# neonbjb/tortoise-tts

Hardware: NVIDIA H100
Metric: audio-seconds/sec at preset='standard' (higher is better)
Workload: dtype bf16 tensor-core operands, fp32 accumulate/residual/norm/softmax/scheduler

## Files before the change

### tortoise_tts_b200/csrc/common.cuh

```cuda
#pragma once
#include <cuda_runtime.h>
#include <cuda_bf16.h>
#include <cuda.h>
#include <stdint.h>
#include <cstdlib>

#define TTB_DEVINL __device__ __forceinline__

namespace ttb {

void set_error(const char* fmt, ...);
int check_cuda(cudaError_t e, const char* what);
#define TTB_CHECK_LAUNCH(what)                                   \
  do {                                                           \
    cudaError_t _e = cudaGetLastError();                         \
    if (_e != cudaSuccess) return ttb::check_cuda(_e, what);     \
  } while (0)

TTB_DEVINL void pdl_wait() { asm volatile("griddepcontrol.wait;" ::: "memory"); }
TTB_DEVINL void pdl_launch_dependents() { asm volatile("griddepcontrol.launch_dependents;" ::: "memory"); }

inline bool pdl_enabled() {
  static int v = -1;
  if (v < 0) {
// ... 46 lines not shown
  __syncthreads();
  if (lane == 0) red[w] = v;
  __syncthreads();
  float r = (lane < nw) ? red[lane] : 0.f;
  r = warp_sum(r);
  return r;
}
TTB_DEVINL float block_max(float v, float* red) {
  int lane = threadIdx.x & 31, w = threadIdx.x >> 5, nw = (blockDim.x + 31) >> 5;
  v = warp_max(v);
  __syncthreads();
  if (lane == 0) red[w] = v;
  __syncthreads();
  float r = (lane < nw) ? red[lane] : -INFINITY;
  r = warp_max(r);
  return r;
}

TTB_DEVINL uint32_t pack_bf16(float a, float b) {
  __nv_bfloat162 t = __floats2bfloat162_rn(a, b);
  return *reinterpret_cast<uint32_t*>(&t);
}
TTB_DEVINL float2 unpack_bf16(uint32_t u) {
  __nv_bfloat162 t = *reinterpret_cast<__nv_bfloat162*>(&u);
  return __bfloat1622float2(t);
}

TTB_DEVINL uint32_t smem_u32(const void* p) { return static_cast<uint32_t>(__cvta_generic_to_shared(p)); }

TTB_DEVINL unsigned long long global_timer_ns() {
  unsigned long long t;
  asm volatile("mov.u64 %0, %%globaltimer;" : "=l"(t));
  return t;
}
TTB_DEVINL unsigned long long sm_id() {
  uint32_t s;
  asm volatile("mov.u32 %0, %%smid;" : "=r"(s));
  return s;
}

TTB_DEVINL bool elect_one() {
  uint32_t pred = 0;
  asm volatile(
      "{\n\t.reg .pred P;\n\t.reg .b32 R;\n\t"
      "elect.sync R|P, 0xffffffff;\n\t"
      "selp.u32 %0, 1, 0, P;\n\t}\n"
      : "=r"(pred));
  return pred != 0;
}

TTB_DEVINL void mbar_init(uint64_t* bar, uint32_t count) {
  asm volatile("mbarrier.init.shared::cta.b64 [%0], %1;" ::"r"(smem_u32(bar)), "r"(count));
}
TTB_DEVINL void fence_barrier_init() { asm volatile("fence.mbarrier_init.release.cluster;" ::: "memory"); }
TTB_DEVINL void fence_proxy_async() { asm volatile("fence.proxy.async.shared::cta;" ::: "memory"); }
TTB_DEVINL void mbar_arrive_expect_tx(uint64_t* bar, uint32_t bytes) {
  asm volatile("mbarrier.arrive.expect_tx.shared::cta.b64 _, [%0], %1;" ::"r"(smem_u32(bar)), "r"(bytes) : "memory");
}
TTB_DEVINL void mbar_arrive(uint64_t* bar) {
  asm volatile("mbarrier.arrive.shared::cta.b64 _, [%0];" ::"r"(smem_u32(bar)) : "memory");
}
#ifndef TTB_MBAR_HINT_NS
#define TTB_MBAR_HINT_NS 20000
#endif
TTB_DEVINL void mbar_wait(uint64_t* bar, uint32_t parity) {
#if TTB_MBAR_HINT_NS > 0
  asm volatile(
      "{\n\t.reg .pred P1;\n\t"
      "WAIT_LOOP:\n\t"
      "mbarrier.try_wait.parity.shared::cta.b64 P1, [%0], %1, %2;\n\t"
      "@P1 bra DONE;\n\t"
      "bra WAIT_LOOP;\n\t"
      "DONE:\n\t}\n" ::"r"(smem_u32(bar)),
      "r"(parity), "r"((uint32_t)TTB_MBAR_HINT_NS)
      : "memory");
#else
  asm volatile(
      "{\n\t.reg .pred P1;\n\t"
      "WAIT_LOOP:\n\t"
      "mbarrier.try_wait.parity.shared::cta.b64 P1, [%0], %1;\n\t"
      "@P1 bra DONE;\n\t"
      "bra WAIT_LOOP;\n\t"
      "DONE:\n\t}\n" ::"r"(smem_u32(bar)),
      "r"(parity)
      : "memory");
#endif
}

TTB_DEVINL void tma_prefetch_desc(const CUtensorMap* m) {
  asm volatile("prefetch.tensormap [%0];" ::"l"(reinterpret_cast<uint64_t>(m)) : "memory");
}
TTB_DEVINL void tma_load_2d(void* smem_dst, const CUtensorMap* map, uint64_t* bar, int c0, int c1) {
  asm volatile(
      "cp.async.bulk.tensor.2d.shared::cluster.global.mbarrier::complete_tx::bytes [%0], [%1, {%3, %4}], [%2];"
      ::"r"(smem_u32(smem_dst)), "l"(reinterpret_cast<uint64_t>(map)), "r"(smem_u32(bar)), "r"(c0), "r"(c1)
      : "memory");
}
TTB_DEVINL void tma_load_3d(void* smem_dst, const CUtensorMap* map, uint64_t* bar, int c0, int c1, int c2) {
  asm volatile(
      "cp.async.bulk.tensor.3d.shared::cluster.global.mbarrier::complete_tx::bytes [%0], [%1, {%3, %4, %5}], [%2];"
      ::"r"(smem_u32(smem_dst)), "l"(reinterpret_cast<uint64_t>(map)), "r"(smem_u32(bar)), "r"(c0), "r"(c1), "r"(c2)
      : "memory");
}
TTB_DEVINL void tma_prefetch_l2_3d(const CUtensorMap* map, int c0, int c1, int c2) {
  asm volatile("cp.async.bulk.prefetch.tensor.3d.L2.global.tile [%0, {%1, %2, %3}];"
               ::"l"(reinterpret_cast<uint64_t>(map)), "r"(c0), "r"(c1), "r"(c2)
               : "memory");
}

TTB_DEVINL void wgmma_fence() { asm volatile("wgmma.fence.sync.aligned;" ::: "memory"); }
TTB_DEVINL void wgmma_commit() { asm volatile("wgmma.commit_group.sync.aligned;" ::: "memory"); }
template <int N>
TTB_DEVINL void wgmma_wait() { asm volatile("wgmma.wait_group.sync.aligned %0;" ::"n"(N) : "memory"); }
TTB_DEVINL void named_barrier(int id, int nthreads) { asm volatile("bar.sync %0, %1;" ::"r"(id), "r"(nthreads) : "memory"); }

TTB_DEVINL uint64_t wgmma_desc_kmajor_sw128(uint32_t smem_addr) {
  uint64_t d = 0;
  d |= (uint64_t)((smem_addr & 0x3FFFF) >> 4);
  d |= (uint64_t)1 << 16;
  d |= (uint64_t)(1024 >> 4) << 32;
  d |= (uint64_t)1 << 62;
  return d;
}
TTB_DEVINL uint64_t wgmma_desc_mnmajor_sw128(uint32_t smem_addr, uint32_t lbo_bytes) {
  uint64_t d = 0;
  d |= (uint64_t)((smem_addr & 0x3FFFF) >> 4);
  d |= (uint64_t)((lbo_bytes >> 4) & 0x3FFF) << 16;
  d |= (uint64_t)(1024 >> 4) << 32;
  d |= (uint64_t)1 << 62;
  return d;
}

TTB_DEVINL void wgmma_m64n16k16_bf16_ss(float* d, uint64_t desc_a, uint64_t desc_b, uint32_t scale_d) {
  asm volatile(
      "{\n\t.reg .pred p;\n\tsetp.ne.b32 p, %10, 0;\n\t"
      "wgmma.mma_async.sync.aligned.m64n16k16.f32.bf16.bf16 {%0, %1, %2, %3, %4, %5, %6, %7}, %8, %9, p, 1, 1, 0, 0;\n\t}\n"
      : "+f"(d[0]), "+f"(d[1]), "+f"(d[2]), "+f"(d[3]), "+f"(d[4]), "+f"(d[5]), "+f"(d[6]), "+f"(d[7])
      : "l"(desc_a), "l"(desc_b), "r"(scale_d));
}
TTB_DEVINL void wgmma_m64n32k16_bf16_ss(float* d, uint64_t desc_a, uint64_t desc_b, uint32_t scale_d) {
  asm volatile(
      "{\n\t.reg .pred p;\n\tsetp.ne.b32 p, %18, 0;\n\t"
      "wgmma.mma_async.sync.aligned.m64n32k16.f32.bf16.bf16 {%0, %1, %2, %3, %4, %5, %6, %7, %8, %9, %10, %11, %12, %13, %14, %15}, %16, %17, p, 1, 1, 0, 0;\n\t}\n"
      : "+f"(d[0]), "+f"(d[1]), "+f"(d[2]), "+f"(d[3]), "+f"(d[4]), "+f"(d[5]), "+f"(d[6]), "+f"(d[7]), "+f"(d[8]), "+f"(d[9]), "+f"(d[10]), "+f"(d[11]), "+f"(d[12]), "+f"(d[13]), "+f"(d[14]), "+f"(d[15])
      : "l"(desc_a), "l"(desc_b), "r"(scale_d));
}
TTB_DEVINL void wgmma_m64n64k16_bf16_ss(float* d, uint64_t desc_a, uint64_t desc_b, uint32_t scale_d) {
  asm volatile(
      "{\n\t.reg .pred p;\n\tsetp.ne.b32 p, %34, 0;\n\t"
      "wgmma.mma_async.sync.aligned.m64n64k16.f32.bf16.bf16 {%0, %1, %2, %3, %4, %5, %6, %7, %8, %9, %10, %11, %12, %13, %14, %15, %16, %17, %18, %19, %20, %21, %22, %23, %24, %25, %26, %27, %28, %29, %30, %31}, %32, %33, p, 1, 1, 0, 0;\n\t}\n"
      : "+f"(d[0]), "+f"(d[1]), "+f"(d[2]), "+f"(d[3]), "+f"(d[4]), "+f"(d[5]), "+f"(d[6]), "+f"(d[7]), "+f"(d[8]), "+f"(d[9]), "+f"(d[10]), "+f"(d[11]), "+f"(d[12]), "+f"(d[13]), "+f"(d[14]), "+f"(d[15]), "+f"(d[16]), "+f"(d[17]), "+f"(d[18]), "+f"(d[19]), "+f"(d[20]), "+f"(d[21]), "+f"(d[22]), "+f"(d[23]), "+f"(d[24]), "+f"(d[25]), "+f"(d[26]), "+f"(d[27]), "+f"(d[28]), "+f"(d[29]), "+f"(d[30]), "+f"(d[31])
      : "l"(desc_a), "l"(desc_b), "r"(scale_d));
}
template <int TNSPB>
TTB_DEVINL void wgmma_m64n64k16_bf16_rs(float* d, const uint32_t* a, uint64_t desc_b, uint32_t scale_d) {
  asm volatile(
      "{\n\t.reg .pred p;\n\tsetp.ne.b32 p, %37, 0;\n\t"
      "wgmma.mma_async.sync.aligned.m64n64k16.f32.bf16.bf16 {%0, %1, %2, %3, %4, %5, %6, %7, %8, %9, %10, %11, %12, %13, %14, %15, %16, %17, %18, %19, %20, %21, %22, %23, %24, %25, %26, %27, %28, %29, %30, %31}, {%32, %33, %34, %35}, %36, p, 1, 1, %38;\n\t}\n"
      : "+f"(d[0]), "+f"(d[1]), "+f"(d[2]), "+f"(d[3]), "+f"(d[4]), "+f"(d[5]), "+f"(d[6]), "+f"(d[7]), "+f"(d[8]), "+f"(d[9]), "+f"(d[10]), "+f"(d[11]), "+f"(d[12]), "+f"(d[13]), "+f"(d[14]), "+f"(d[15]), "+f"(d[16]), "+f"(d[17]), "+f"(d[18]), "+f"(d[19]), "+f"(d[20]), "+f"(d[21]), "+f"(d[22]), "+f"(d[23]), "+f"(d[24]), "+f"(d[25]), "+f"(d[26]), "+f"(d[27]), "+f"(d[28]), "+f"(d[29]), "+f"(d[30]), "+f"(d[31])
      : "r"(a[0]), "r"(a[1]), "r"(a[2]), "r"(a[3]), "l"(desc_b), "r"(scale_d), "n"(TNSPB));
}

template <int BN>
TTB_DEVINL void gemm_mma_kblock(float* acc, uint32_t sa, uint32_t sb, bool first) {
  wgmma_fence();
#pragma unroll
  for (int k = 0; k < 4; ++k) {
    const uint64_t da = wgmma_desc_kmajor_sw128(sa + k * 32);
    const uint32_t sc = (first && k == 0) ? 0u : 1u;
    if constexpr (BN == 32) {
      wgmma_m64n32k16_bf16_ss(acc, da, wgmma_desc_kmajor_sw128(sb + k * 32), sc);
    } else {
#pragma unroll
      for (int nb = 0; nb < BN / 64; ++nb)
        wgmma_m64n64k16_bf16_ss(acc + nb * 32, da, wgmma_desc_kmajor_sw128(sb + nb * 8192 + k * 32), sc);
    }
  }
  wgmma_commit();
}

}
```

### tortoise_tts_b200/csrc/gemm.cu

```cuda
#include "common.cuh"
#include "ttb_internal.h"

#include <map>
#include <mutex>
#include <string>
#include <vector>
#include <cstring>

namespace ttb {

typedef CUresult (*PFN_encodeTiled)(CUtensorMap*, CUtensorMapDataType, cuuint32_t, void*, const cuuint64_t*,
                                    const cuuint64_t*, const cuuint32_t*, const cuuint32_t*, CUtensorMapInterleave,
                                    CUtensorMapSwizzle, CUtensorMapL2promotion, CUtensorMapFloatOOBfill);

static PFN_encodeTiled get_encode_fn() {
  static PFN_encodeTiled fn = nullptr;
  static std::once_flag once;
  std::call_once(once, []() {
    void* p = nullptr;
    cudaDriverEntryPointQueryResult q;
    if (cudaGetDriverEntryPoint("cuTensorMapEncodeTiled", &p, cudaEnableDefault, &q) == cudaSuccess &&
        q == cudaDriverEntryPointSuccess)
      fn = reinterpret_cast<PFN_encodeTiled>(p);
  });
// ... 158 lines not shown
          tma_load_3d(sb, &map_b, &full_bar[kbi], tap * K + kk, n0, 0);
        } else if (ep.wpre > 1) {
          tma_prefetch_l2_3d(&map_b, tap * K + kk, n0, 0);
        } else {
          break;
        }
      }
    }
  }
  pdl_wait();
  if (tr && threadIdx.x == 0) tr[2] = global_timer_ns();

  if (warp == PRODUCER_WARP) {
    if (lane == 0 || (SPLIT_PRODUCER && lane == 1)) {
      int stage = 0; uint32_t phase = 0;
      for (int kbi = 0; kbi < pre; ++kbi) {
        const int kb = kb_begin + kbi;
        const int tap = kb / kblocks_per_tap;
        const int kk = (kb - tap * kblocks_per_tap) * BK;
        tma_load_3d(smem + kbi * L::STAGE_BYTES, &map_a, &full_bar[kbi], kk, m0 + tap * ep.tap_dil - pad, bz * a_batch_mul);
        if (++stage == STAGES) { stage = 0; phase ^= 1; }
      }
      for (int kbi = pre; kbi < num_kb; ++kbi) {
        mbar_wait(&empty_bar[stage], phase ^ 1);
        const int kb = kb_begin + kbi;
        const int tap = kb / kblocks_per_tap;
        const int kk = (kb - tap * kblocks_per_tap) * BK;
        uint8_t* sa = smem + stage * L::STAGE_BYTES;
        uint8_t* sb = sa + L::A_BYTES;
        if constexpr (SPLIT_PRODUCER) {
          if (lane == 0) {
            mbar_arrive_expect_tx(&full_bar[stage], L::A_BYTES);
            tma_load_3d(sa, &map_a, &full_bar[stage], kk, m0 + tap * ep.tap_dil - pad, bz * a_batch_mul);
          } else {
            mbar_arrive_expect_tx(&full_bar[stage], L::B_BYTES);
            tma_load_3d(sb, &map_b, &full_bar[stage], tap * K + kk, n0, 0);
          }
        } else {
          mbar_arrive_expect_tx(&full_bar[stage], L::STAGE_BYTES);
          tma_load_3d(sa, &map_a, &full_bar[stage], kk, m0 + tap * ep.tap_dil - pad, bz * a_batch_mul);
          tma_load_3d(sb, &map_b, &full_bar[stage], tap * K + kk, n0, 0);
        }
        if (++stage == STAGES) { stage = 0; phase ^= 1; }
      }
    }
    __syncwarp();
    pdl_launch_dependents();
  } else {
    const int wg = warp >> 2;
    const int rb = warp >> 1;
    if (ep.residual) {
      const int m = m0 + rb * 32 + lane;
      if (m < M && !(warp & 1)) {
        const float* p = ep.residual + (long long)bz * ep.res_bstride + (long long)m * ep.ldr + n0;
#pragma unroll
        for (int c = 0; c < BN; c += 32)
          if (n0 + c < N) asm volatile("prefetch.global.L2 [%0];" ::"l"(p + c));
      }
    }
    float acc[BN / 2];
    int stage = 0; uint32_t phase = 0;
    if (tr && threadIdx.x == 0) tr[3] = global_timer_ns();
    gemm_consumer_mainloop<BN, STAGES>(acc, smem, L::STAGE_BYTES, L::A_BYTES, full_bar, empty_bar, num_kb, stage, phase, wg,
                                       (threadIdx.x & 127) == 0, [](uint64_t* b) { mbar_arrive(b); });
    if (tr && threadIdx.x == 0) tr[4] = global_timer_ns();
    pdl_launch_dependents();
    named_barrier(1, GEMM_CONSUMERS);
    gemm_stage_accumulator<BN>(acc, smem_u32(smem), warp, lane);
    named_barrier(1, GEMM_CONSUMERS);
    if (tr && threadIdx.x == 0) tr[5] = global_timer_ns();
    gemm_epilogue_dispatch<BN>(smem_u32(smem) + (uint32_t)(rb * 32 * (BN + 8)) * 4, n0, N, m0 + rb * 32, M, lane, (long long)bz,
                               ep, warp & 1, 2);
    if (tr && threadIdx.x == 0) tr[6] = global_timer_ns();
  }
  __syncthreads();
  if (tr && threadIdx.x == 0) tr[7] = global_timer_ns();
}

__global__ void gemm_ref_kernel(const __nv_bfloat16* A, long long a_bstride, int lda, int rows, const __nv_bfloat16* W,
                                int M, int N, int K, int taps, int pad, GemmEpilogue ep) {
  const int n = blockIdx.x * blockDim.x + threadIdx.x;
  const int m = blockIdx.y;
  const int bz = blockIdx.z;
  if (n >= N || m >= M) return;
  const int nn = (ep.act == TTB_ACT_GEGLU) ? (n & ~1) : n;
  float acc[2] = {0.f, 0.f};
  const int cnt = (ep.act == TTB_ACT_GEGLU) ? 2 : 1;
  if (ep.act == TTB_ACT_GEGLU && (n & 1)) return;
  for (int c = 0; c < cnt; ++c) {
    float s = 0.f;
    for (int tap = 0; tap < taps; ++tap) {
      const int r = m + tap - pad;
      if (r < 0 || r >= rows) continue;
      const __nv_bfloat16* a = A + (long long)bz * a_bstride + (long long)r * lda;
      const __nv_bfloat16* w = W + (long long)(nn + c) * taps * K + (long long)tap * K;
      for (int k = 0; k < K; ++k) s += __bfloat162float(a[k]) * __bfloat162float(w[k]);
    }
    s *= ep.alpha;
    if (ep.bias) s += ep.bias[nn + c];
    acc[c] = s;
  }
  float v;
  int on = n;
  if (ep.act == TTB_ACT_GEGLU) { v = acc[0] * gelu_erf(acc[1]); on = n >> 1; }
  else {
    v = acc[0];
    if (ep.act == TTB_ACT_GELU_NEW) v = gelu_new(v);
    else if (ep.act == TTB_ACT_SILU) v = silu(v);
    else if (ep.act == TTB_ACT_LRELU02) v = leaky(v, 0.2f);
    else if (ep.act == TTB_ACT_GELU_ERF) v = gelu_erf(v);
    if (ep.residual) v += ep.residual[(long long)bz * ep.res_bstride + (long long)m * ep.ldr + n];
  }
  if (ep.out_f32) ep.out_f32[(long long)bz * ep.outf_bstride + (long long)m * ep.ldo + on] = v;
  if (ep.out_bf16) ep.out_bf16[(long long)bz * ep.outb_bstride + (long long)m * ep.ldob + on] = __float2bfloat16(v);
}

static int g_gemm_impl = -1;
static unsigned long long* g_gemm_trace = nullptr;

template <int BN, int STAGES, bool SPLIT_PRODUCER = false>
static int launch_tc(const TtbGemmArgs& g, const GemmEpilogue& ep, cudaStream_t st) {
  CUtensorMap ma, mb;
  const bool bcast = (g.batch == 1) || (g.a_bstride == 0);
  const uint64_t a_d2 = bcast ? 1 : (uint64_t)g.batch;
  const uint64_t a_s2 = bcast ? (uint64_t)g.rows * g.lda : (uint64_t)g.a_bstride;
  if (get_tensor_map_bf16(&ma, g.A, (uint64_t)g.K, (uint64_t)g.rows, a_d2, (uint64_t)g.lda, a_s2, BK, BM)) return -1;
  if (get_tensor_map_bf16(&mb, g.W, (uint64_t)g.K * g.taps, (uint64_t)g.N, 1, (uint64_t)g.K * g.taps,
                          (uint64_t)g.K * g.taps * g.N, BK, BN)) return -1;
  using L = GemmSmem<BN, STAGES>;
  static bool attr_set = false;
  if (!attr_set) {
    cudaError_t e = cudaFuncSetAttribute(gemm_bf16_tc_kernel<BN, STAGES, SPLIT_PRODUCER>, cudaFuncAttributeMaxDynamicSharedMemorySize, L::TOTAL);
    if (e != cudaSuccess) return check_cuda(e, "cudaFuncSetAttribute(gemm)");
    attr_set = true;
  }
  int kb_per_split = 0, zdim = g.batch;
  if (g.splitk > 1) {
    const int kb_total = (g.K / BK) * g.taps;
    kb_per_split = (kb_total + g.splitk - 1) / g.splitk;
    zdim = (kb_total + kb_per_split - 1) / kb_per_split;
  }
  dim3 grid((g.N + BN - 1) / BN, (g.M + BM - 1) / BM, zdim);
  cudaError_t le = launch_pdl(gemm_bf16_tc_kernel<BN, STAGES, SPLIT_PRODUCER>, grid, dim3(GEMM_THREADS), (size_t)L::TOTAL, st, ma, mb, g.M, g.N,
                              g.K, g.taps, g.pad, (bcast || g.splitk > 1) ? 0 : 1, kb_per_split, ep, g_gemm_trace);
  if (le != cudaSuccess) return check_cuda(le, "gemm_bf16_tc_kernel launch");
  TTB_CHECK_LAUNCH("gemm_bf16_tc_kernel");
  return 0;
}

}

#include "gemm_persist.cuh"
#include "gemm_mc.cuh"

namespace ttb {

static int num_sms() {
  static int n = 0;
  if (!n) {
    int dev = 0;
    cudaGetDevice(&dev);
    cudaDeviceGetAttribute(&n, cudaDevAttrMultiProcessorCount, dev);
    if (n <= 0) n = 132;
  }
  return n;
}

template <int BN, int PSTAGES>
static int launch_persistent(const TtbGemmArgs& g, const GemmEpilogue& ep, cudaStream_t st) {
  CUtensorMap ma, mb;
  const bool bcast = (g.batch == 1) || (g.a_bstride == 0);
  const uint64_t a_d2 = bcast ? 1 : (uint64_t)g.batch;
  const uint64_t a_s2 = bcast ? (uint64_t)g.rows * g.lda : (uint64_t)g.a_bstride;
  if (get_tensor_map_bf16(&ma, g.A, (uint64_t)g.K, (uint64_t)g.rows, a_d2, (uint64_t)g.lda, a_s2, BK, BM)) return -1;
  if (get_tensor_map_bf16(&mb, g.W, (uint64_t)g.K * g.taps, (uint64_t)g.N, 1, (uint64_t)g.K * g.taps,
                          (uint64_t)g.K * g.taps * g.N, BK, BN)) return -1;
  using L = GemmPSmem<BN, PSTAGES>;
  static bool attr_set = false;
  if (!attr_set) {
    cudaError_t e = cudaFuncSetAttribute(gemm_bf16_tc_persistent_kernel<BN, PSTAGES>,
                                         cudaFuncAttributeMaxDynamicSharedMemorySize, L::TOTAL);
    if (e != cudaSuccess) return check_cuda(e, "cudaFuncSetAttribute(gemm persistent)");
    attr_set = true;
  }
  int kb_per_split = 0, zdim = g.batch;
  if (g.splitk > 1) {
    const int kb_total = (g.K / BK) * g.taps;
    kb_per_split = (kb_total + g.splitk - 1) / g.splitk;
    zdim = (kb_total + kb_per_split - 1) / kb_per_split;
  }
  const int m_tiles = (g.M + BM - 1) / BM, n_tiles = (g.N + BN - 1) / BN;
  const long long total = (long long)m_tiles * n_tiles * zdim;
  const int grid = (int)(total < num_sms() ? total : num_sms());
  const cudaError_t le = launch_pdl(gemm_bf16_tc_persistent_kernel<BN, PSTAGES>, dim3(grid), dim3(GEMM_THREADS), (size_t)L::TOTAL, st,
      ma, mb, g.M, g.N, g.K, g.taps, g.pad, (bcast || g.splitk > 1) ? 0 : 1, kb_per_split, m_tiles, n_tiles, zdim, ep);
  if (le != cudaSuccess) return check_cuda(le, "gemm_bf16_tc_persistent_kernel launch");
  TTB_CHECK_LAUNCH("gemm_bf16_tc_persistent_kernel");
  return 0;
}

}

using namespace ttb;

extern "C" int ttb_debug_gemm_trace(void* buf) {
  g_gemm_trace = static_cast<unsigned long long*>(buf);
  return 0;
}

extern "C" int ttb_gemm(const TtbGemmArgs* gp, void* stream) {
  const TtbGemmArgs& g = *gp;
  cudaStream_t st = static_cast<cudaStream_t>(stream);
  if (g.K % BK != 0 || g.K <= 0) { set_error("ttb_gemm: K=%d must be a positive multiple of 64", g.K); return -1; }
  if (g.taps < 1 || g.M <= 0 || g.N <= 0 || g.batch <= 0) { set_error("ttb_gemm: bad shape"); return -1; }
  if (g.act == TTB_ACT_GEGLU && (g.N & 1)) { set_error("ttb_gemm: GEGLU needs even N"); return -1; }
  GemmEpilogue ep;
  ep.bias = g.bias; ep.residual = g.residual; ep.out_f32 = g.out_f32;
  ep.out_bf16 = reinterpret_cast<__nv_bfloat16*>(g.out_bf16);
  ep.res_bstride = g.res_bstride; ep.outf_bstride = g.outf_bstride; ep.outb_bstride = g.outb_bstride;
  ep.ldr = g.ldr; ep.ldo = g.ldo; ep.ldob = g.ldob; ep.act = g.act; ep.alpha = g.alpha;
  ep.gn_part = nullptr; ep.gn_groups = g.gn_groups;
  static int wpre_on = -1;
  if (wpre_on < 0) { const char* e = getenv("TTB_GEMM_WPREFETCH"); wpre_on = e ? atoi(e) : 1; }
  ep.wpre = g.w_static ? wpre_on : 0;
  ep.tap_dil = g.tap_dilation > 1 ? g.tap_dilation : 1;
  if (ep.tap_dil > 1 && (g.cluster > 1 || g.variant == 6 || g.force_ref || g_gemm_impl == 1)) {
    set_error("ttb_gemm: tap_dilation is implemented by the one-tile and the persistent kernels only");
    return -1;
  }
  if (g.gn_partials) {
    if (g.N != 32 * g.gn_groups || (g.M + 31) / 32 > TTB_GN_SPLITS || g.act == TTB_ACT_GEGLU || g.splitk > 1 || g.force_ref) {
      set_error("ttb_gemm: gn_partials needs N == 32 * gn_groups, M <= %d, no GEGLU / split-K (N=%d groups=%d M=%d)",
                32 * TTB_GN_SPLITS, g.N, g.gn_groups, g.M);
      return -1;
    }
    ep.gn_part = reinterpret_cast<float2*>(g.gn_partials + 16);
  }
  if (g_gemm_impl < 0) {
    const char* e = getenv("TTB_GEMM_IMPL");
    g_gemm_impl = (e && strcmp(e, "ref") == 0) ? 1 : 0;
  }
  if (g.splitk > 1) {
    if (g.batch != 1 || g.act != TTB_ACT_NONE || !g.out_f32 || g.out_bf16 || g.bias || g.residual) {
      set_error("ttb_gemm: splitk needs batch=1, no activation/bias/residual and an fp32 partial buffer");
      return -1;
    }
    if (g_gemm_impl == 1 || g.force_ref) { set_error("ttb_gemm: splitk is not available in the SIMT checker"); return -1; }
  }
  if (g_gemm_impl == 1 || g.force_ref) {
    dim3 block(128), grid((g.N + 127) / 128, g.M, g.batch);
    gemm_ref_kernel<<<grid, block, 0, st>>>(reinterpret_cast<const __nv_bfloat16*>(g.A), g.a_bstride, g.lda, g.rows,
                                            reinterpret_cast<const __nv_bfloat16*>(g.W), g.M, g.N, g.K, g.taps, g.pad, ep);
    TTB_CHECK_LAUNCH("gemm_ref_kernel");
    return 0;
  }
  const long long tiles128 = (long long)((g.N + 127) / 128) * ((g.M + BM - 1) / BM) * g.batch;
  if (g.cluster > 1) {
    const int bn = g.tile_n == 32 ? 32 : (g.tile_n == 64 ? 64 : 128);
    const int n_tiles = (g.N + bn - 1) / bn;
    if ((g.cluster != 2 && g.cluster != 4) || n_tiles % g.cluster != 0) {
      set_error("ttb_gemm: cluster=%d needs 2 or 4 and a multiple of it in N tiles (%d)", g.cluster, n_tiles);
      return -1;
    }
    if (bn == 32) return g.cluster == 4 ? launch_mc<32, 4, 4>(g, ep, st) : launch_mc<32, 4, 2>(g, ep, st);
    if (bn == 64) return g.cluster == 4 ? launch_mc<64, 4, 4>(g, ep, st) : launch_mc<64, 4, 2>(g, ep, st);
    return g.cluster == 4 ? launch_mc<128, 3, 4>(g, ep, st) : launch_mc<128, 3, 2>(g, ep, st);
  }
  if (g.variant == 6) { set_error("ttb_gemm: variant 6 (CTA-pair MMA) needs hardware this library does not target"); return -1; }
  static int persist = -1;
  if (persist < 0) { const char* e = getenv("TTB_GEMM_PERSIST"); persist = e ? atoi(e) : 0; }
  if (g.variant == 2) {
    if (g.tile_n == 32) return launch_persistent<32, 8>(g, ep, st);
    if (g.tile_n == 64) return launch_persistent<64, 6>(g, ep, st);
    return launch_persistent<128, 4>(g, ep, st);
  }
  const int use_persist = (g.variant == 1) ? 0 : persist;
  if (use_persist && g.tile_n == 0 && tiles128 >= 2 * num_sms()) return launch_persistent<128, 4>(g, ep, st);
  if (use_persist == 2) {
    if (g.tile_n == 32) return launch_persistent<32, 8>(g, ep, st);
    if (g.tile_n == 64 || (g.tile_n == 0 && tiles128 < num_sms())) return launch_persistent<64, 6>(g, ep, st);
    if (g.tile_n != 256) return launch_persistent<128, 4>(g, ep, st);
  }
  if (g.tile_n == 32) {
    static int t32 = -1;
    if (t32 < 0) { const char* e = getenv("TTB_GEMM_T32_STAGES"); t32 = e ? atoi(e) : 5; }
    return (g.variant == 3 || (g.variant != 4 && t32 == 5)) ? launch_tc<32, 5>(g, ep, st) : launch_tc<32, 4>(g, ep, st);
  }
  if (g.tile_n == 64 && g.variant == 3) return launch_tc<64, 8>(g, ep, st);
  if (g.tile_n == 64 || (g.tile_n == 0 && tiles128 < num_sms())) return launch_tc<64, 4>(g, ep, st);
  if (g.tile_n == 256) return launch_tc<256, 3>(g, ep, st);
  if (g.variant == 5) return launch_tc<128, 3, true>(g, ep, st);
  return launch_tc<128, 3>(g, ep, st);
}
```

### tortoise_tts_b200/csrc/gemm_epilogue.cuh

```cuda
#pragma once

namespace ttb {

TTB_DEVINL float4 lds128(uint32_t addr) {
  float4 v;
  asm volatile("ld.shared.v4.f32 {%0, %1, %2, %3}, [%4];" : "=f"(v.x), "=f"(v.y), "=f"(v.z), "=f"(v.w) : "r"(addr) : "memory");
  return v;
}

template <int BN>
TTB_DEVINL void gemm_stage_accumulator(const float* acc, uint32_t tile, int cwarp, int lane) {
  constexpr int PITCH = BN + 8;
  const uint32_t base = tile + (uint32_t)((cwarp * 16 + (lane >> 2)) * PITCH + 2 * (lane & 3)) * 4;
#pragma unroll
  for (int i = 0; i < BN / 2; i += 4) {
    asm volatile("st.shared.v2.f32 [%0], {%1, %2};" ::"r"(base + (uint32_t)(2 * i) * 4), "f"(acc[i]), "f"(acc[i + 1]) : "memory");
    asm volatile("st.shared.v2.f32 [%0], {%1, %2};" ::"r"(base + (uint32_t)(8 * PITCH + 2 * i) * 4), "f"(acc[i + 2]), "f"(acc[i + 3]) : "memory");
  }
}

template <int ACT>
TTB_DEVINL float epi_act(float x) {
  if (ACT == TTB_ACT_GELU_NEW) return gelu_new(x);
  if (ACT == TTB_ACT_SILU) return silu(x);
  if (ACT == TTB_ACT_LRELU02) return leaky(x, 0.2f);
  if (ACT == TTB_ACT_TANH) return tanhf(x);
  if (ACT == TTB_ACT_GELU_ERF) return gelu_erf(x);
  return x;
}

struct EpiFlags {
  bool aligned;
};

TTB_DEVINL EpiFlags epi_flags(const GemmEpilogue& ep) {
  EpiFlags f;
  f.aligned = (!ep.bias || (reinterpret_cast<uintptr_t>(ep.bias) & 15) == 0) &&
              (!ep.residual || ((ep.ldr & 3) == 0 && (ep.res_bstride & 3) == 0 && (reinterpret_cast<uintptr_t>(ep.residual) & 15) == 0)) &&
              (!ep.out_f32 || ((ep.ldo & 3) == 0 && (ep.outf_bstride & 3) == 0 && (reinterpret_cast<uintptr_t>(ep.out_f32) & 15) == 0)) &&
              (!ep.out_bf16 || ((ep.ldob & 3) == 0 && (ep.outb_bstride & 3) == 0 && (reinterpret_cast<uintptr_t>(ep.out_bf16) & 7) == 0));
  return f;
}

TTB_DEVINL void epi_gn_store(float gs, float gq, int nb, int m_base, int lane, long long bz, const GemmEpilogue& ep) {
#pragma unroll
  for (int off = 16; off > 0; off >>= 1) {
    gs += __shfl_xor_sync(0xffffffffu, gs, off);
    gq += __shfl_xor_sync(0xffffffffu, gq, off);
  }
  if (lane == 0)
    ep.gn_part[((long long)bz * ep.gn_groups + (nb >> 5)) * TTB_GN_SPLITS + (m_base >> 5)] = make_float2(gs, gq);
}

template <int ACT>
TTB_DEVINL void epi_chunk_fast(uint32_t blk, int pitch, int nb, int m_base, int rows_valid, int lane, long long bz,
                               const GemmEpilogue& ep) {
  const bool GN = ep.gn_part != nullptr;
  const int rr0 = lane >> 3, c = (lane & 7) * 4;
  float4 b = make_float4(0.f, 0.f, 0.f, 0.f);
  if (ep.bias) b = __ldg(reinterpret_cast<const float4*>(ep.bias + nb + c));
  if (ACT == TTB_ACT_GEGLU) {
    const long long col = (nb >> 1) + (c >> 1);
#pragma unroll
    for (int it = 0; it < 8; ++it) {
      const int rr = it * 4 + rr0;
      const float4 a = lds128(blk + (uint32_t)(rr * pitch + c) * 4);
      const float o0 = fmaf(a.x, ep.alpha, b.x) * gelu_erf(fmaf(a.y, ep.alpha, b.y));
      const float o1 = fmaf(a.z, ep.alpha, b.z) * gelu_erf(fmaf(a.w, ep.alpha, b.w));
      const long long m = m_base + rr;
      if (rr >= rows_valid) continue;
      if (ep.out_bf16) *reinterpret_cast<uint32_t*>(ep.out_bf16 + bz * ep.outb_bstride + m * ep.ldob + col) = pack_bf16(o0, o1);
      if (ep.out_f32) *reinterpret_cast<float2*>(ep.out_f32 + bz * ep.outf_bstride + m * ep.ldo + col) = make_float2(o0, o1);
    }
    return;
  }
  const long long col = nb + c;
  float4 rs[8];
  if (ep.residual) {
    const float* rp = ep.residual + bz * ep.res_bstride + (long long)(m_base + rr0) * ep.ldr + col;
#pragma unroll
    for (int it = 0; it < 8; ++it) {
      if (it * 4 + rr0 < rows_valid) rs[it] = *reinterpret_cast<const float4*>(rp + (long long)it * 4 * ep.ldr);
      else rs[it] = make_float4(0.f, 0.f, 0.f, 0.f);
    }
  }
  float gs = 0.f, gq = 0.f;
#pragma unroll
  for (int it = 0; it < 8; ++it) {
    const int rr = it * 4 + rr0;
    const float4 a = lds128(blk + (uint32_t)(rr * pitch + c) * 4);
    float4 o;
    o.x = epi_act<ACT>(fmaf(a.x, ep.alpha, b.x));
    o.y = epi_act<ACT>(fmaf(a.y, ep.alpha, b.y));
    o.z = epi_act<ACT>(fmaf(a.z, ep.alpha, b.z));
    o.w = epi_act<ACT>(fmaf(a.w, ep.alpha, b.w));
    if (ep.residual) { o.x += rs[it].x; o.y += rs[it].y; o.z += rs[it].z; o.w += rs[it].w; }
    const long long m = m_base + rr;
    if (rr >= rows_valid) continue;
    if (ep.out_f32) *reinterpret_cast<float4*>(ep.out_f32 + bz * ep.outf_bstride + m * ep.ldo + col) = o;
    if (ep.out_bf16)
      *reinterpret_cast<uint2*>(ep.out_bf16 + bz * ep.outb_bstride + m * ep.ldob + col) = make_uint2(pack_bf16(o.x, o.y), pack_bf16(o.z, o.w));
    if (GN) {
      gs += (o.x + o.y) + (o.z + o.w);
      gq += (o.x * o.x + o.y * o.y) + (o.z * o.z + o.w * o.w);
    }
  }
  if (GN) epi_gn_store(gs, gq, nb, m_base, lane, bz, ep);
}

template <int ACT>
TTB_DEVINL void epi_chunk_slow(const uint32_t* r, int nb, int N, int m, int M, long long bz, const GemmEpilogue& ep,
                               float& gs, float& gq) {
  if (m >= M) return;
  if (ACT == TTB_ACT_GEGLU) {
    const int nout = N >> 1, ob = nb >> 1;
    float* of = ep.out_f32 ? ep.out_f32 + bz * ep.outf_bstride + (long long)m * ep.ldo : nullptr;
    __nv_bfloat16* obf = ep.out_bf16 ? ep.out_bf16 + bz * ep.outb_bstride + (long long)m * ep.ldob : nullptr;
#pragma unroll
    for (int j = 0; j < 16; ++j) {
      if (ob + j < nout) {
        float u = __uint_as_float(r[2 * j]) * ep.alpha, g = __uint_as_float(r[2 * j + 1]) * ep.alpha;
        if (ep.bias) { u += __ldg(ep.bias + nb + 2 * j); g += __ldg(ep.bias + nb + 2 * j + 1); }
        const float o = u * gelu_erf(g);
        if (of) of[ob + j] = o;
        if (obf) obf[ob + j] = __float2bfloat16(o);
      }
    }
    return;
  }
  const float* rp = ep.residual ? ep.residual + bz * ep.res_bstride + (long long)m * ep.ldr : nullptr;
  float* of = ep.out_f32 ? ep.out_f32 + bz * ep.outf_bstride + (long long)m * ep.ldo : nullptr;
  __nv_bfloat16* obf = ep.out_bf16 ? ep.out_bf16 + bz * ep.outb_bstride + (long long)m * ep.ldob : nullptr;
#pragma unroll
  for (int j = 0; j < 32; ++j) {
    if (nb + j < N) {
      float x = __uint_as_float(r[j]) * ep.alpha;
      if (ep.bias) x += __ldg(ep.bias + nb + j);
      x = epi_act<ACT>(x);
      if (rp) x += rp[nb + j];
      if (of) of[nb + j] = x;
      if (obf) obf[nb + j] = __float2bfloat16(x);
      gs += x;
      gq += x * x;
    }
  }
}

template <int BN, int ACT>
TTB_DEVINL void gemm_epilogue_tile(uint32_t blk, int n0, int N, int m_base, int M, int lane, long long bz,
                                   const GemmEpilogue& ep, int ch_begin, int ch_step) {
  constexpr int NCH = BN / 32;
  constexpr int PITCH = BN + 8;
  const bool aligned = epi_flags(ep).aligned;
  const int rows_valid = min(32, M - m_base);
#pragma unroll 1
  for (int ch = ch_begin; ch < NCH; ch += ch_step) {
    const int nb = n0 + ch * 32;
    if (nb >= N || rows_valid <= 0) continue;
    if (aligned && nb + 32 <= N) {
      epi_chunk_fast<ACT>(blk + (uint32_t)ch * 128, PITCH, nb, m_base, rows_valid, lane, bz, ep);
    } else {
      uint32_t r[32];
#pragma unroll
      for (int j = 0; j < 8; ++j) {
        const float4 a = lds128(blk + (uint32_t)(lane * PITCH + ch * 32 + 4 * j) * 4);
        r[4 * j] = __float_as_uint(a.x); r[4 * j + 1] = __float_as_uint(a.y);
        r[4 * j + 2] = __float_as_uint(a.z); r[4 * j + 3] = __float_as_uint(a.w);
      }
      float gs = 0.f, gq = 0.f;
      epi_chunk_slow<ACT>(r, nb, N, m_base + lane, M, bz, ep, gs, gq);
      if (ep.gn_part) epi_gn_store(gs, gq, nb, m_base, lane, bz, ep);
    }
  }
}

template <int BN>
TTB_DEVINL void gemm_epilogue_dispatch(uint32_t blk, int n0, int N, int m_base, int M, int lane, long long bz,
                                       const GemmEpilogue& ep, int ch_begin, int ch_step) {
  switch (ep.act) {
    case TTB_ACT_GEGLU: gemm_epilogue_tile<BN, TTB_ACT_GEGLU>(blk, n0, N, m_base, M, lane, bz, ep, ch_begin, ch_step); break;
    case TTB_ACT_GELU_NEW: gemm_epilogue_tile<BN, TTB_ACT_GELU_NEW>(blk, n0, N, m_base, M, lane, bz, ep, ch_begin, ch_step); break;
    case TTB_ACT_SILU: gemm_epilogue_tile<BN, TTB_ACT_SILU>(blk, n0, N, m_base, M, lane, bz, ep, ch_begin, ch_step); break;
    case TTB_ACT_LRELU02: gemm_epilogue_tile<BN, TTB_ACT_LRELU02>(blk, n0, N, m_base, M, lane, bz, ep, ch_begin, ch_step); break;
    case TTB_ACT_TANH: gemm_epilogue_tile<BN, TTB_ACT_TANH>(blk, n0, N, m_base, M, lane, bz, ep, ch_begin, ch_step); break;
    case TTB_ACT_GELU_ERF: gemm_epilogue_tile<BN, TTB_ACT_GELU_ERF>(blk, n0, N, m_base, M, lane, bz, ep, ch_begin, ch_step); break;
    default: gemm_epilogue_tile<BN, TTB_ACT_NONE>(blk, n0, N, m_base, M, lane, bz, ep, ch_begin, ch_step); break;
  }
}

}
```

Measured before the change: 6.990.

## Add warp-specialised persistent 128x256 WGMMA GEMM with register reallocation

Adds a persistent, warp-specialised GEMM kernel. One producer warpgroup issues TMA loads, while two consumer warpgroups each run m64n256k16 WGMMA across a 4-stage mbarrier pipeline. setmaxnreg moves registers from the producer to the consumers. The epilogue is staged through shared memory in 32-column slices. The kernel is on by default for non-split-K GEMMs whose 128x128 tile count fills the SMs; it aims to improve tensor-core utilisation and overlap loads with MMA. The cost is heavy register pressure from 128 accumulator floats per thread, and an epilogue that does not overlap with the next tile's mainloop.

After: 7.380 (median of 6 runs). 1.06x the previous value.

```diff
diff --git a/tortoise_tts_b200/csrc/common.cuh b/tortoise_tts_b200/csrc/common.cuh
--- a/tortoise_tts_b200/csrc/common.cuh
+++ b/tortoise_tts_b200/csrc/common.cuh
@@ -222,6 +222,13 @@
       : "+f"(d[0]), "+f"(d[1]), "+f"(d[2]), "+f"(d[3]), "+f"(d[4]), "+f"(d[5]), "+f"(d[6]), "+f"(d[7]), "+f"(d[8]), "+f"(d[9]), "+f"(d[10]), "+f"(d[11]), "+f"(d[12]), "+f"(d[13]), "+f"(d[14]), "+f"(d[15]), "+f"(d[16]), "+f"(d[17]), "+f"(d[18]), "+f"(d[19]), "+f"(d[20]), "+f"(d[21]), "+f"(d[22]), "+f"(d[23]), "+f"(d[24]), "+f"(d[25]), "+f"(d[26]), "+f"(d[27]), "+f"(d[28]), "+f"(d[29]), "+f"(d[30]), "+f"(d[31])
       : "l"(desc_a), "l"(desc_b), "r"(scale_d));
 }
+TTB_DEVINL void wgmma_m64n256k16_bf16_ss(float* d, uint64_t desc_a, uint64_t desc_b, uint32_t scale_d) {
+  asm volatile(
+      "{\n\t.reg .pred p;\n\tsetp.ne.b32 p, %130, 0;\n\t"
+      "wgmma.mma_async.sync.aligned.m64n256k16.f32.bf16.bf16 {%0, %1, %2, %3, %4, %5, %6, %7, %8, %9, %10, %11, %12, %13, %14, %15, %16, %17, %18, %19, %20, %21, %22, %23, %24, %25, %26, %27, %28, %29, %30, %31, %32, %33, %34, %35, %36, %37, %38, %39, %40, %41, %42, %43, %44, %45, %46, %47, %48, %49, %50, %51, %52, %53, %54, %55, %56, %57, %58, %59, %60, %61, %62, %63, %64, %65, %66, %67, %68, %69, %70, %71, %72, %73, %74, %75, %76, %77, %78, %79, %80, %81, %82, %83, %84, %85, %86, %87, %88, %89, %90, %91, %92, %93, %94, %95, %96, %97, %98, %99, %100, %101, %102, %103, %104, %105, %106, %107, %108, %109, %110, %111, %112, %113, %114, %115, %116, %117, %118, %119, %120, %121, %122, %123, %124, %125, %126, %127}, %128, %129, p, 1, 1, 0, 0;\n\t}\n"
+      : "+f"(d[0]), "+f"(d[1]), "+f"(d[2]), "+f"(d[3]), "+f"(d[4]), "+f"(d[5]), "+f"(d[6]), "+f"(d[7]), "+f"(d[8]), "+f"(d[9]), "+f"(d[10]), "+f"(d[11]), "+f"(d[12]), "+f"(d[13]), "+f"(d[14]), "+f"(d[15]), "+f"(d[16]), "+f"(d[17]), "+f"(d[18]), "+f"(d[19]), "+f"(d[20]), "+f"(d[21]), "+f"(d[22]), "+f"(d[23]), "+f"(d[24]), "+f"(d[25]), "+f"(d[26]), "+f"(d[27]), "+f"(d[28]), "+f"(d[29]), "+f"(d[30]), "+f"(d[31]), "+f"(d[32]), "+f"(d[33]), "+f"(d[34]), "+f"(d[35]), "+f"(d[36]), "+f"(d[37]), "+f"(d[38]), "+f"(d[39]), "+f"(d[40]), "+f"(d[41]), "+f"(d[42]), "+f"(d[43]), "+f"(d[44]), "+f"(d[45]), "+f"(d[46]), "+f"(d[47]), "+f"(d[48]), "+f"(d[49]), "+f"(d[50]), "+f"(d[51]), "+f"(d[52]), "+f"(d[53]), "+f"(d[54]), "+f"(d[55]), "+f"(d[56]), "+f"(d[57]), "+f"(d[58]), "+f"(d[59]), "+f"(d[60]), "+f"(d[61]), "+f"(d[62]), "+f"(d[63]), "+f"(d[64]), "+f"(d[65]), "+f"(d[66]), "+f"(d[67]), "+f"(d[68]), "+f"(d[69]), "+f"(d[70]), "+f"(d[71]), "+f"(d[72]), "+f"(d[73]), "+f"(d[74]), "+f"(d[75]), "+f"(d[76]), "+f"(d[77]), "+f"(d[78]), "+f"(d[79]), "+f"(d[80]), "+f"(d[81]), "+f"(d[82]), "+f"(d[83]), "+f"(d[84]), "+f"(d[85]), "+f"(d[86]), "+f"(d[87]), "+f"(d[88]), "+f"(d[89]), "+f"(d[90]), "+f"(d[91]), "+f"(d[92]), "+f"(d[93]), "+f"(d[94]), "+f"(d[95]), "+f"(d[96]), "+f"(d[97]), "+f"(d[98]), "+f"(d[99]), "+f"(d[100]), "+f"(d[101]), "+f"(d[102]), "+f"(d[103]), "+f"(d[104]), "+f"(d[105]), "+f"(d[106]), "+f"(d[107]), "+f"(d[108]), "+f"(d[109]), "+f"(d[110]), "+f"(d[111]), "+f"(d[112]), "+f"(d[113]), "+f"(d[114]), "+f"(d[115]), "+f"(d[116]), "+f"(d[117]), "+f"(d[118]), "+f"(d[119]), "+f"(d[120]), "+f"(d[121]), "+f"(d[122]), "+f"(d[123]), "+f"(d[124]), "+f"(d[125]), "+f"(d[126]), "+f"(d[127])
+      : "l"(desc_a), "l"(desc_b), "r"(scale_d));
+}
 template <int TNSPB>
 TTB_DEVINL void wgmma_m64n64k16_bf16_rs(float* d, const uint32_t* a, uint64_t desc_b, uint32_t scale_d) {
   asm volatile(
@@ -249,4 +256,19 @@
   wgmma_commit();
 }
 
-}
+TTB_DEVINL void gemm_mma_kblock_n256(float* acc, uint32_t sa, uint32_t sb, bool first) {
+  wgmma_fence();
+#pragma unroll
+  for (int k = 0; k < 4; ++k)
+    wgmma_m64n256k16_bf16_ss(acc, wgmma_desc_kmajor_sw128(sa + k * 32), wgmma_desc_kmajor_sw128(sb + k * 32),
+                             (first && k == 0) ? 0u : 1u);
+  wgmma_commit();
+}
+
+template <int R>
+TTB_DEVINL void setmaxnreg_dec() { asm volatile("setmaxnreg.dec.sync.aligned.u32 %0;" ::"n"(R)); }
+template <int R>
+TTB_DEVINL void setmaxnreg_inc() { asm volatile("setmaxnreg.inc.sync.aligned.u32 %0;" ::"n"(R)); }
+
+
+}
diff --git a/tortoise_tts_b200/csrc/gemm.cu b/tortoise_tts_b200/csrc/gemm.cu
--- a/tortoise_tts_b200/csrc/gemm.cu
+++ b/tortoise_tts_b200/csrc/gemm.cu
@@ -334,6 +334,7 @@
 
 #include "gemm_persist.cuh"
 #include "gemm_mc.cuh"
+#include "gemm_ws.cuh"
 
 namespace ttb {
 
@@ -378,6 +379,30 @@
       ma, mb, g.M, g.N, g.K, g.taps, g.pad, (bcast || g.splitk > 1) ? 0 : 1, kb_per_split, m_tiles, n_tiles, zdim, ep);
   if (le != cudaSuccess) return check_cuda(le, "gemm_bf16_tc_persistent_kernel launch");
   TTB_CHECK_LAUNCH("gemm_bf16_tc_persistent_kernel");
+  return 0;
+}
+
+static int launch_ws(const TtbGemmArgs& g, const GemmEpilogue& ep, cudaStream_t st) {
+  CUtensorMap ma, mb;
+  const bool bcast = (g.batch == 1) || (g.a_bstride == 0);
+  const uint64_t a_d2 = bcast ? 1 : (uint64_t)g.batch;
+  const uint64_t a_s2 = bcast ? (uint64_t)g.rows * g.lda : (uint64_t)g.a_bstride;
+  if (get_tensor_map_bf16(&ma, g.A, (uint64_t)g.K, (uint64_t)g.rows, a_d2, (uint64_t)g.lda, a_s2, BK, BM)) return -1;
+  if (get_tensor_map_bf16(&mb, g.W, (uint64_t)g.K * g.taps, (uint64_t)g.N, 1, (uint64_t)g.K * g.taps,
+                          (uint64_t)g.K * g.taps * g.N, BK, WS_BN)) return -1;
+  static bool attr_set = false;
+  if (!attr_set) {
+    cudaError_t e = cudaFuncSetAttribute(gemm_bf16_ws_kernel, cudaFuncAttributeMaxDynamicSharedMemorySize, GemmWsSmem::TOTAL);
+    if (e != cudaSuccess) return check_cuda(e, "cudaFuncSetAttribute(gemm ws)");
+    attr_set = true;
+  }
+  const int m_tiles = (g.M + BM - 1) / BM, n_tiles = (g.N + WS_BN - 1) / WS_BN;
+  const long long total = (long long)m_tiles * n_tiles * g.batch;
+  const int grid = (int)(total < num_sms() ? total : num_sms());
+  const cudaError_t le = launch_pdl(gemm_bf16_ws_kernel, dim3(grid), dim3(WS_THREADS), (size_t)GemmWsSmem::TOTAL, st,
+      ma, mb, g.M, g.N, g.K, g.taps, g.pad, bcast ? 0 : 1, m_tiles, n_tiles, g.batch, ep);
+  if (le != cudaSuccess) return check_cuda(le, "gemm_bf16_ws_kernel launch");
+  TTB_CHECK_LAUNCH("gemm_bf16_ws_kernel");
   return 0;
 }
 
@@ -449,6 +474,10 @@
     return g.cluster == 4 ? launch_mc<128, 3, 4>(g, ep, st) : launch_mc<128, 3, 2>(g, ep, st);
   }
   if (g.variant == 6) { set_error("ttb_gemm: variant 6 (CTA-pair MMA) needs hardware this library does not target"); return -1; }
+  if (g.variant == 7) {
+    if (g.splitk > 1) { set_error("ttb_gemm: variant 7 (warp-specialised 128x256) has no split-K"); return -1; }
+    return launch_ws(g, ep, st);
+  }
   static int persist = -1;
   if (persist < 0) { const char* e = getenv("TTB_GEMM_PERSIST"); persist = e ? atoi(e) : 0; }
   if (g.variant == 2) {
@@ -463,6 +492,9 @@
     if (g.tile_n == 64 || (g.tile_n == 0 && tiles128 < num_sms())) return launch_persistent<64, 6>(g, ep, st);
     if (g.tile_n != 256) return launch_persistent<128, 4>(g, ep, st);
   }
+  static int ws = -1;
+  if (ws < 0) { const char* e = getenv("TTB_GEMM_WS"); ws = e ? atoi(e) : 1; }
+  if (ws && g.tile_n == 0 && g.variant == 0 && g.splitk <= 1 && tiles128 >= num_sms()) return launch_ws(g, ep, st);
   if (g.tile_n == 32) {
     static int t32 = -1;
     if (t32 < 0) { const char* e = getenv("TTB_GEMM_T32_STAGES"); t32 = e ? atoi(e) : 5; }
diff --git a/tortoise_tts_b200/csrc/gemm_epilogue.cuh b/tortoise_tts_b200/csrc/gemm_epilogue.cuh
--- a/tortoise_tts_b200/csrc/gemm_epilogue.cuh
+++ b/tortoise_tts_b200/csrc/gemm_epilogue.cuh
@@ -8,9 +8,8 @@
   return v;
 }
 
-template <int BN>
+template <int BN, int PITCH = BN + 8>
 TTB_DEVINL void gemm_stage_accumulator(const float* acc, uint32_t tile, int cwarp, int lane) {
-  constexpr int PITCH = BN + 8;
   const uint32_t base = tile + (uint32_t)((cwarp * 16 + (lane >> 2)) * PITCH + 2 * (lane & 3)) * 4;
 #pragma unroll
   for (int i = 0; i < BN / 2; i += 4) {
@@ -146,11 +145,10 @@
   }
 }
 
-template <int BN, int ACT>
+template <int BN, int ACT, int PITCH = BN + 8>
 TTB_DEVINL void gemm_epilogue_tile(uint32_t blk, int n0, int N, int m_base, int M, int lane, long long bz,
                                    const GemmEpilogue& ep, int ch_begin, int ch_step) {
   constexpr int NCH = BN / 32;
-  constexpr int PITCH = BN + 8;
   const bool aligned = epi_flags(ep).aligned;
   const int rows_valid = min(32, M - m_base);
 #pragma unroll 1
@@ -174,17 +172,17 @@
   }
 }
 
-template <int BN>
+template <int BN, int PITCH = BN + 8>
 TTB_DEVINL void gemm_epilogue_dispatch(uint32_t blk, int n0, int N, int m_base, int M, int lane, long long bz,
                                        const GemmEpilogue& ep, int ch_begin, int ch_step) {
   switch (ep.act) {
-    case TTB_ACT_GEGLU: gemm_epilogue_tile<BN, TTB_ACT_GEGLU>(blk, n0, N, m_base, M, lane, bz, ep, ch_begin, ch_step); break;
-    case TTB_ACT_GELU_NEW: gemm_epilogue_tile<BN, TTB_ACT_GELU_NEW>(blk, n0, N, m_base, M, lane, bz, ep, ch_begin, ch_step); break;
-    case TTB_ACT_SILU: gemm_epilogue_tile<BN, TTB_ACT_SILU>(blk, n0, N, m_base, M, lane, bz, ep, ch_begin, ch_step); break;
-    case TTB_ACT_LRELU02: gemm_epilogue_tile<BN, TTB_ACT_LRELU02>(blk, n0, N, m_base, M, lane, bz, ep, ch_begin, ch_step); break;
-    case TTB_ACT_TANH: gemm_epilogue_tile<BN, TTB_ACT_TANH>(blk, n0, N, m_base, M, lane, bz, ep, ch_begin, ch_step); break;
-    case TTB_ACT_GELU_ERF: gemm_epilogue_tile<BN, TTB_ACT_GELU_ERF>(blk, n0, N, m_base, M, lane, bz, ep, ch_begin, ch_step); break;
-    default: gemm_epilogue_tile<BN, TTB_ACT_NONE>(blk, n0, N, m_base, M, lane, bz, ep, ch_begin, ch_step); break;
+    case TTB_ACT_GEGLU: gemm_epilogue_tile<BN, TTB_ACT_GEGLU, PITCH>(blk, n0, N, m_base, M, lane, bz, ep, ch_begin, ch_step); break;
+    case TTB_ACT_GELU_NEW: gemm_epilogue_tile<BN, TTB_ACT_GELU_NEW, PITCH>(blk, n0, N, m_base, M, lane, bz, ep, ch_begin, ch_step); break;
+    case TTB_ACT_SILU: gemm_epilogue_tile<BN, TTB_ACT_SILU, PITCH>(blk, n0, N, m_base, M, lane, bz, ep, ch_begin, ch_step); break;
+    case TTB_ACT_LRELU02: gemm_epilogue_tile<BN, TTB_ACT_LRELU02, PITCH>(blk, n0, N, m_base, M, lane, bz, ep, ch_begin, ch_step); break;
+    case TTB_ACT_TANH: gemm_epilogue_tile<BN, TTB_ACT_TANH, PITCH>(blk, n0, N, m_base, M, lane, bz, ep, ch_begin, ch_step); break;
+    case TTB_ACT_GELU_ERF: gemm_epilogue_tile<BN, TTB_ACT_GELU_ERF, PITCH>(blk, n0, N, m_base, M, lane, bz, ep, ch_begin, ch_step); break;
+    default: gemm_epilogue_tile<BN, TTB_ACT_NONE, PITCH>(blk, n0, N, m_base, M, lane, bz, ep, ch_begin, ch_step); break;
   }
 }
 
diff --git a/tortoise_tts_b200/csrc/gemm_ws.cuh b/tortoise_tts_b200/csrc/gemm_ws.cuh
--- /dev/null
+++ b/tortoise_tts_b200/csrc/gemm_ws.cuh
@@ -0,0 +1,148 @@
+#pragma once
+
+namespace ttb {
+
+constexpr int WS_BN = 256;
+constexpr int WS_STAGES = 4;
+constexpr int WS_THREADS = 384;
+constexpr int WS_SLICE = 32;
+
+struct GemmWsSmem {
+  static constexpr int A_BYTES = BM * BK * 2;
+  static constexpr int B_BYTES = WS_BN * BK * 2;
+  static constexpr int STAGE_BYTES = A_BYTES + B_BYTES;
+  static constexpr int STG_PITCH = WS_SLICE;
+  static constexpr int SLICE_BYTES = 64 * STG_PITCH * 4;
+  static constexpr int STG_OFF = WS_STAGES * STAGE_BYTES;
+  static constexpr int BAR_OFF = STG_OFF + 4 * SLICE_BYTES;
+  static constexpr int TOTAL = BAR_OFF + 2 * WS_STAGES * 8 + 1024;
+  static_assert(TOTAL <= 227 * 1024, "warp-specialised GEMM shared memory");
+};
+
+__global__ void __launch_bounds__(WS_THREADS, 1)
+gemm_bf16_ws_kernel(const __grid_constant__ CUtensorMap map_a, const __grid_constant__ CUtensorMap map_b, int M, int N,
+                    int K, int taps, int pad, int a_batch_mul, int m_tiles, int n_tiles, int z_tiles, GemmEpilogue ep) {
+  extern __shared__ uint8_t smem_raw[];
+  uint8_t* smem = reinterpret_cast<uint8_t*>((reinterpret_cast<uintptr_t>(smem_raw) + 1023) & ~uintptr_t(1023));
+  using L = GemmWsSmem;
+  uint64_t* full_bar = reinterpret_cast<uint64_t*>(smem + L::BAR_OFF);
+  uint64_t* empty_bar = full_bar + WS_STAGES;
+
+  const int warp = threadIdx.x >> 5;
+  const int lane = threadIdx.x & 31;
+  const int kblocks_per_tap = K / BK;
+  const int num_kb = kblocks_per_tap * taps;
+  const int total_tiles = m_tiles * n_tiles * z_tiles;
+
+  if (threadIdx.x == 0) {
+    tma_prefetch_desc(&map_a);
+    tma_prefetch_desc(&map_b);
+    for (int s = 0; s < WS_STAGES; ++s) { mbar_init(&full_bar[s], 1); mbar_init(&empty_bar[s], 2); }
+    fence_barrier_init();
+  }
+  __syncthreads();
+  int pre = 0;
+  if (ep.wpre && threadIdx.x == 0) {
+    const int n0 = ((blockIdx.x / m_tiles) % n_tiles) * WS_BN;
+    pre = num_kb < WS_STAGES ? num_kb : WS_STAGES;
+    for (int kb = 0; kb < num_kb; ++kb) {
+      const int tap = kb / kblocks_per_tap;
+      const int kk = (kb - tap * kblocks_per_tap) * BK;
+      if (kb < pre) {
+        mbar_arrive_expect_tx(&full_bar[kb], L::STAGE_BYTES);
+        tma_load_3d(smem + kb * L::STAGE_BYTES + L::A_BYTES, &map_b, &full_bar[kb], tap * K + kk, n0, 0);
+      } else if (ep.wpre > 1) {
+        tma_prefetch_l2_3d(&map_b, tap * K + kk, n0, 0);
+      } else {
+        break;
+      }
+    }
+  }
+  pdl_wait();
+
+  if (warp < 4) {
+    setmaxnreg_dec<40>();
+    if (threadIdx.x == 0) {
+      int stage = 0; uint32_t phase = 0;
+      for (int tile = blockIdx.x; tile < total_tiles; tile += gridDim.x) {
+        const int mt = tile % m_tiles, rest = tile / m_tiles;
+        const int nt = rest % n_tiles, bz = rest / n_tiles;
+        const int m0 = mt * BM, n0 = nt * WS_BN;
+        const int npre = tile == (int)blockIdx.x ? pre : 0;
+        for (int kb = 0; kb < num_kb; ++kb) {
+          const int tap = kb / kblocks_per_tap;
+          const int kk = (kb - tap * kblocks_per_tap) * BK;
+          uint8_t* sa = smem + stage * L::STAGE_BYTES;
+          if (kb >= npre) {
+            mbar_wait(&empty_bar[stage], phase ^ 1);
+            mbar_arrive_expect_tx(&full_bar[stage], L::STAGE_BYTES);
+            tma_load_3d(sa + L::A_BYTES, &map_b, &full_bar[stage], tap * K + kk, n0, 0);
+          }
+          tma_load_3d(sa, &map_a, &full_bar[stage], kk, m0 + tap * ep.tap_dil - pad, bz * a_batch_mul);
+          if (++stage == WS_STAGES) { stage = 0; phase ^= 1; }
+        }
+      }
+    }
+    __syncwarp();
+    pdl_launch_dependents();
+  } else {
+    setmaxnreg_inc<232>();
+    const int cw = warp - 4;
+    const int wg = cw >> 2;
+    const int rb = cw >> 1;
+    const bool leader = (threadIdx.x & 127) == 0;
+    const uint32_t stg = smem_u32(smem + L::STG_OFF) + (uint32_t)(wg * 2 * L::SLICE_BYTES);
+    const uint32_t blk = stg + (uint32_t)((cw & 1) * L::SLICE_BYTES + (rb & 1) * 32 * L::STG_PITCH * 4);
+    int stage = 0; uint32_t phase = 0;
+    float acc[WS_BN / 2];
+    for (int tile = blockIdx.x; tile < total_tiles; tile += gridDim.x) {
+      const int mt = tile % m_tiles, rest = tile / m_tiles;
+      const int nt = rest % n_tiles, bz = rest / n_tiles;
+      const int m0 = mt * BM, n0 = nt * WS_BN;
+      if (ep.residual && !(cw & 1)) {
+        const int m = m0 + rb * 32 + lane;
+        if (m < M) {
+          const float* p = ep.residual + (long long)bz * ep.res_bstride + (long long)m * ep.ldr + n0;
+#pragma unroll
+          for (int c = 0; c < WS_BN; c += 32)
+            if (n0 + c < N) asm volatile("prefetch.global.L2 [%0];" ::"l"(p + c));
+        }
+      }
+      int prev = -1;
+      for (int kb = 0; kb < num_kb; ++kb) {
+        mbar_wait(&full_bar[stage], phase);
+        const uint32_t sa = smem_u32(smem + stage * L::STAGE_BYTES);
+        gemm_mma_kblock_n256(acc, sa + wg * (64 * BK * 2), sa + L::A_BYTES, kb == 0);
+        wgmma_wait<1>();
+        if (prev >= 0 && leader) mbar_arrive(&empty_bar[prev]);
+        prev = stage;
+        if (++stage == WS_STAGES) { stage = 0; phase ^= 1; }
+      }
+      wgmma_wait<0>();
+      if (leader) mbar_arrive(&empty_bar[prev]);
+      if (tile + (int)gridDim.x >= total_tiles) pdl_launch_dependents();
+#pragma unroll 1
+      for (int r = 0; r < WS_BN / (2 * WS_SLICE); ++r) {
+        if (n0 + r * 2 * WS_SLICE >= N) break;
+        named_barrier(1 + wg, 128);
+#pragma unroll
+        for (int j = 0; j < WS_BN / (2 * WS_SLICE); ++j) {
+          if (j == r) {
+            gemm_stage_accumulator<WS_SLICE, L::STG_PITCH>(acc + 2 * j * (WS_SLICE / 2), stg, cw & 3, lane);
+            gemm_stage_accumulator<WS_SLICE, L::STG_PITCH>(acc + (2 * j + 1) * (WS_SLICE / 2), stg + L::SLICE_BYTES, cw & 3, lane);
+          }
+        }
+        named_barrier(1 + wg, 128);
+        const int nb = n0 + (2 * r + (cw & 1)) * WS_SLICE;
+        if (nb < N) {
+          int mb = m0 + rb * 32, ln = lane, b = bz;
+          uint32_t bk = blk;
+          asm volatile("" : "+r"(mb), "+r"(ln), "+r"(b), "+r"(bk));
+          gemm_epilogue_dispatch<WS_SLICE, L::STG_PITCH>(bk, nb, N, mb, M, ln, (long long)b, ep, 0, 1);
+        }
+      }
+    }
+  }
+}
+
+}
```
